# alexbuburuzan/MObI

Measured on AMD Instinct MI355X. Metric: denoising throughput (UNet element-forwards/s = steps/s x UNet batch), higher is better.
Workload: dtype bf16; 1 GPU; mobi_nusc_512 UNet denoising step, 8 objects/GPU (UNet batch 16), latent 64x64, DDIM-50 schedule, cfg_scale 1.0; objects_per_gpu=8, unet_batch=16, latent=64, sampler=ddim, parallelism=dp1 (objects sharded, no collective in the loop)

## Files before the change

mobi_amd/csrc/igemm.hip:

```cpp
#include <stdlib.h>

#include <type_traits>

#include "common.h"
#include "tuning.h"
#include "igemm_small.h"

#ifndef MOBI_FRAG2
#define MOBI_FRAG2 0
#endif
#ifndef MOBI_DMA_KS
#define MOBI_DMA_KS 1
#endif
#if defined(MOBI_IGEMM_FENCE) && MOBI_IGEMM_FENCE
#define MOBI_SCHED_FENCE() __builtin_amdgcn_sched_barrier(0)
#else
#define MOBI_SCHED_FENCE() ((void)0)
#endif

#ifndef MOBI_DBG_SKIP
#define MOBI_DBG_SKIP 0
#endif
#ifndef MOBI_PP_DMA_KS
#define MOBI_PP_DMA_KS 1
// ... 37 lines not shown
__device__ unsigned long long* g_phase = nullptr;
#define MOBI_PHASE_DECL unsigned long long ph_t[6]; unsigned ph_acc[5] = {0u, 0u, 0u, 0u, 0u}; unsigned ph_n = 0
#define MOBI_PHASE(i) ph_t[i] = __builtin_amdgcn_s_memrealtime()
#define MOBI_PHASE_ACC()                                                                  \
  do {                                                                                    \
    for (int i_ = 0; i_ < 5; ++i_) ph_acc[i_] += (unsigned)(ph_t[i_ + 1] - ph_t[i_]);     \
    ++ph_n;                                                                               \
  } while (0)
#else
#define MOBI_PHASE_DECL ((void)0)
#define MOBI_PHASE(i) ((void)0)
#define MOBI_PHASE_ACC() ((void)0)
#endif

#if MOBI_STAMP == 5
#define MOBI_SP_ENTRY const unsigned long long sp_t0 = __builtin_amdgcn_s_memtime()
#define MOBI_SP_DECL unsigned long long sp_t[7], sp_acc[6] = {0, 0, 0, 0, 0, 0}, sp_n = 0, sp_first = 0, sp_last = 0
#define MOBI_SP(i) sp_t[i] = __builtin_amdgcn_s_memtime()
#define MOBI_SP_ACC()                                                              \
  do {                                                                             \
    for (int i_ = 0; i_ < 6; ++i_) sp_acc[i_] += sp_t[i_ + 1] - sp_t[i_];          \
    if (!sp_n) sp_first = sp_t[0];                                                 \
    sp_last = sp_t[6];                                                             \
    ++sp_n;                                                                        \
  } while (0)
#define MOBI_SP_WRITE()                                                                                                   \
  do {                                                                                                                    \
    asm volatile("s_waitcnt vmcnt(0)" ::: "memory");                                                                      \
    const unsigned long long sp_end = __builtin_amdgcn_s_memtime();                                                       \
    if (g_phase && lane == 0) {                                                                                           \
      unsigned long long* d_ = g_phase + ((size_t)(blockIdx.x + gridDim.x * (blockIdx.y + gridDim.y * blockIdx.z)) * 8 + wave * 2) * 8; \
      for (int i_ = 0; i_ < 6; ++i_) d_[i_] = sp_acc[i_];                                                                 \
      d_[6] = sp_n; d_[7] = sp_end - sp_t0;                                                                               \
      d_[8] = sp_n ? sp_first - sp_t0 : 0; d_[9] = sp_n ? sp_end - sp_last : 0;                                           \
    }                                                                                                                     \
  } while (0)
#else
#define MOBI_SP_ENTRY ((void)0)
#define MOBI_SP_DECL ((void)0)
#define MOBI_SP(i) ((void)0)
#define MOBI_SP_ACC() ((void)0)
#define MOBI_SP_WRITE() ((void)0)
#endif

__device__ __attribute__((aligned(16))) unsigned int g_zero16[4] = {0u, 0u, 0u, 0u};

struct IgemmArgs {
  const void* src0; const void* src1;
  int c0, c1, C;
  int hin, win, up, hout, wout, hw_out;
  int kh, kw, stride, pad_h, pad_w;
  int img_pix_stride;
  const void* weight; long long w_group_stride;
  int n_packed, cout, ktot, nk;
  int M;
  int imgs_per_group;
  const float* bias; const float* rowvec; int rowvec_stride;
  const void* residual; long long res_img_stride;
  void* out; long long out_img_stride;
  int out_mode, epilogue;
  float scale;
  int tiles_m, tiles_n;
  int n_major;
  int src0_bytes, src1_bytes, w_bytes, fast, glds;
  int k_order;
  int wm;
  int splits, nk_per;
  float* split_ws;
  const float* ln_svec;
  float ln_eps;
  int sync_mode;
  int* sync;
  int ring_direct;
  int sm_direct;
  const void* w_tiled;
  int sm64;
  int lin_window;
  int epi_direct;
  int pp;
  int sm;
  int wide;
  int hw_shift, w_shift;
  int small;
};

#define MOBI_TILE_OF_M(L_, tile_m_, tile_n_) const int tile_n_ = (L_) % a.tiles_n, tile_m_ = (L_) / a.tiles_n
#define MOBI_TILE_OF(L_, tile_m_, tile_n_)                                                     \
  const int tdiv_##tile_m_ = __builtin_amdgcn_readfirstlane(a.n_major ? a.tiles_m : a.tiles_n); \
  const int tq_##tile_m_ = (L_) / tdiv_##tile_m_, tr_##tile_m_ = (L_) - tq_##tile_m_ * tdiv_##tile_m_; \
  const int tile_m_ = a.n_major ? tr_##tile_m_ : tq_##tile_m_;                                 \
  const int tile_n_ = a.n_major ? tq_##tile_m_ : tr_##tile_m_


__device__ __forceinline__ void vm_store16_dev(void* p, const u32x4& v);

template <int RPP, bool TR, int NT>
struct EpiGeom {
  static constexpr int WAVE_N = NT * 16;
  static constexpr int STRIDE = TR ? (RPP + 4) : (WAVE_N + 4);
  static constexpr int ROWS = TR ? WAVE_N : RPP;
  static constexpr int BYTES = ROWS * STRIDE * 4;
};

template <typename T, int NT, bool TR, int RPP, bool RES_EARLY = true, bool LEAKY = false>
__device__ __forceinline__ void igemm_epilogue(const IgemmArgs& a, float* stage, f32x4 (&acc)[NT][4], int lane,
                                               int group, int nw0, int mw0) {
  constexpr int WAVE_N = NT * 16;
  constexpr int STAGE_STRIDE = EpiGeom<RPP, TR, NT>::STRIDE;
  constexpr int MT = RPP / 16;
  constexpr int NPASS = 4 / MT;
  const int r16 = lane & 15, g4 = lane >> 4;
  const float scale = a.scale;
  T* __restrict__ outT = reinterpret_cast<T*>(a.out);
  float* __restrict__ outF = reinterpret_cast<float*>(a.out);
  const T* __restrict__ resid = reinterpret_cast<const T*>(a.residual);
  const bool plain = !TR && !a.split_ws && a.epilogue != MOBI_EPI_GEGLU;
  const bool use_bias = a.bias != nullptr && !a.split_ws;

  const int mw0c = mw0 < a.M ? mw0 : 0;
  const int img0 = __builtin_amdgcn_readfirstlane(mw0c / a.hw_out);
  const int rem0 = mw0c - img0 * a.hw_out;
  auto locate = [&](int row_in_tile, int& img, int& rem) {
    img = img0; rem = rem0 + row_in_tile;
    while (rem >= a.hw_out) { rem -= a.hw_out; ++img; }
  };

  f32x4 bias4[NT];
#pragma unroll
  for (int ni = 0; ni < NT; ++ni) {
    bias4[ni] = f32x4{0.f, 0.f, 0.f, 0.f};
    if (use_bias) {
      if (!TR) {
        const int n = nw0 + ni * 16 + g4 * 4;
        if (n < a.n_packed) bias4[ni] = *reinterpret_cast<const f32x4*>(a.bias + n);
      } else {
        const int n = nw0 + ni * 16 + r16;
        const float b = n < a.cout ? a.bias[n] : 0.f;
        bias4[ni] = f32x4{b, b, b, b};
      }
    }
  }

  constexpr int TPR_P = WAVE_N / 8;
  constexpr int NIT_P = (RPP * TPR_P + 63) / 64;
  u32x4 rres[RES_EARLY ? NPASS : 1][NIT_P];
  auto request_rows = [&](int pass, u32x4 (&dst)[NIT_P]) {
#pragma unroll
    for (int it = 0; it < NIT_P; ++it) {
      dst[it] = u32x4{0u, 0u, 0u, 0u};
      const int task = lane + 64 * it;
      const int row = task / TPR_P, cg = task - row * TPR_P;
      const int rt = pass * RPP + row;
      const int n = nw0 + cg * 8;
      if (task < RPP * TPR_P && mw0 + rt < a.M && n < a.cout) {
        int img, rem;
        locate(rt, img, rem);
        const long long gi = (long long)(group * a.imgs_per_group + img);
        dst[it] = ld16(resid + gi * a.res_img_stride + (long long)rem * a.cout + n);
      }
    }
  };
  if (RES_EARLY && plain && resid) {
#pragma unroll
    for (int pass = 0; pass < NPASS; ++pass) request_rows(pass, rres[pass]);
  }

// ... 199 lines not shown
      const int img = m / a.hw_out, rem = m - img * a.hw_out;
      if (a.bias) {
        float bb[8];
        ld8f(a.bias + n, bb);
#pragma unroll
        for (int j = 0; j < 8; ++j) o[j] += bb[j];
      }
      if (a.rowvec) {
        float rv[8];
        ld8f(a.rowvec + (long long)img * a.rowvec_stride + n, rv);
#pragma unroll
        for (int j = 0; j < 8; ++j) o[j] += rv[j];
      }
      if (resid) {
        float rf[8];
        unpack8<T>(ld16(resid + (long long)img * a.res_img_stride + (long long)rem * a.cout + n), rf);
#pragma unroll
        for (int j = 0; j < 8; ++j) o[j] += rf[j];
      }
      const long long off = (long long)img * a.out_img_stride + (long long)rem * a.cout + n;
      if (a.out_mode == MOBI_OUT_ROWS_F32) {
        *reinterpret_cast<f32x4*>(outF + off) = f32x4{o[0], o[1], o[2], o[3]};
        *reinterpret_cast<f32x4*>(outF + off + 4) = f32x4{o[4], o[5], o[6], o[7]};
      } else {
        st16(outT + off, pack8<T>(o));
      }
    }
  }
}

template <typename T, int THREADS>
__device__ __forceinline__ void splitk_arrive_and_finish(const IgemmArgs& a, int tile, int m0, int bm, int n0, int bn, int* s_flag) {
  asm volatile("s_waitcnt vmcnt(0)" ::: "memory");
  __syncthreads();
  if (threadIdx.x == 0) {
    *s_flag = a.sync_mode == 2 ? __hip_atomic_fetch_add(a.sync + tile, 1, __ATOMIC_RELAXED, __HIP_MEMORY_SCOPE_WORKGROUP)
                               : __hip_atomic_fetch_add(a.sync + tile, 1, __ATOMIC_RELAXED, __HIP_MEMORY_SCOPE_AGENT);
  }
  __syncthreads();
  if (*s_flag != a.splits - 1) return;
  if (threadIdx.x == 0) {
    if (a.sync_mode == 2) __hip_atomic_store(a.sync + tile, 0, __ATOMIC_RELAXED, __HIP_MEMORY_SCOPE_WORKGROUP);
    else __hip_atomic_store(a.sync + tile, 0, __ATOMIC_RELAXED, __HIP_MEMORY_SCOPE_AGENT);
  }
  if (a.sync_mode == 2) splitk_finish_tile<T, THREADS, false>(a, m0, bm, n0, bn);
  else splitk_finish_tile<T, THREADS, true>(a, m0, bm, n0, bn);
}

__device__ __forceinline__ void wait_vmcnt_le(int n) {
#define MOBI_VMW(k) else if (n >= k) asm volatile("s_waitcnt vmcnt(" #k ")" ::: "memory")
  if (n >= 37) asm volatile("s_waitcnt vmcnt(37)" ::: "memory");
  MOBI_VMW(32); MOBI_VMW(27); MOBI_VMW(26); MOBI_VMW(22); MOBI_VMW(18); MOBI_VMW(17); MOBI_VMW(14); MOBI_VMW(12);
  MOBI_VMW(10); MOBI_VMW(8); MOBI_VMW(7); MOBI_VMW(6); MOBI_VMW(5); MOBI_VMW(4);
  else asm volatile("s_waitcnt vmcnt(0)" ::: "memory");
#undef MOBI_VMW
}

#ifndef MOBI_PP_GEGLU_STORE16
#define MOBI_PP_GEGLU_STORE16 1
#endif
#ifndef MOBI_PP_WDUP
#define MOBI_PP_WDUP 0
#endif
#ifndef MOBI_PP_FASTWAIT
#define MOBI_PP_FASTWAIT 1
#endif
__device__ __forceinline__ void wait_vmcnt_le_fast(int n) {
  if (!MOBI_PP_FASTWAIT) { wait_vmcnt_le(n); return; }
  if (n == 7) asm volatile("s_waitcnt vmcnt(7)" ::: "memory");
  else if (n == 6) asm volatile("s_waitcnt vmcnt(6)" ::: "memory");
  else wait_vmcnt_le(n);
}

#define MOBI_SWAP4(INSN, X, Y)                                                                                       \
  asm volatile("s_nop 1\n\t" INSN " %0, %4\n\t" INSN " %1, %5\n\t" INSN " %2, %6\n\t" INSN " %3, %7\n\ts_nop 1" \
               : "+v"(X[0]), "+v"(X[1]), "+v"(X[2]), "+v"(X[3]), "+v"(Y[0]), "+v"(Y[1]), "+v"(Y[2]), "+v"(Y[3]))

template <int NT>
struct DirectEpiRegs {
  u32x4 bias[NT];
  u32x4 res[NT][2];
};

template <typename T, int NT, bool VEC = true, bool RES = true>
__device__ __forceinline__ int direct_epilogue_request(const IgemmArgs& a, DirectEpiRegs<NT>& q, int lane, int group,
                                                       int nw0, int mw0) {
  const int r16 = lane & 15, g4 = lane >> 4;
  int n_issued = 0;
  if (VEC && (a.bias || a.rowvec)) {
    const float* vec = a.bias;
    if (a.rowvec) {
      const int img = __builtin_amdgcn_readfirstlane(mw0 / a.hw_out);
      vec = a.rowvec + (long long)(group * a.imgs_per_group + img) * a.rowvec_stride;
    }
#pragma unroll
    for (int ni = 0; ni < NT; ++ni) q.bias[ni] = vm_load16(vec + nw0 + ni * 16 + g4 * 4);
    n_issued += NT;
  }
  if (RES && a.residual) {
    const T* __restrict__ resid = reinterpret_cast<const T*>(a.residual);
#pragma unroll
    for (int p = 0; p < 2; ++p) {
      const int m = mw0 + (2 * p + (g4 & 1)) * 16 + r16;
      const int img = m / a.hw_out, rem = m - img * a.hw_out;
      const T* rowp = resid + (long long)(group * a.imgs_per_group + img) * a.res_img_stride + (long long)rem * a.cout +
                      nw0 + 8 * (g4 >> 1);
#pragma unroll
      for (int ni = 0; ni < NT; ++ni) q.res[ni][p] = vm_load16(rowp + ni * 16);
    }
    n_issued += 2 * NT;
  }
  return n_issued;
}

template <typename T, int NT, bool GEGLU, bool VEC = true>
__device__ __forceinline__ int direct_epilogue(const IgemmArgs& a, f32x4 (&acc)[NT][4], DirectEpiRegs<NT>& q, int lane,
                                               int group, int nw0, int mw0) {
  const int r16 = lane & 15, g4 = lane >> 4;
  const float scale = a.scale;
  T* __restrict__ outT = reinterpret_cast<T*>(a.out);
  const bool has_vec = VEC && (a.bias || a.rowvec);
  if (has_vec) {
#pragma unroll
    for (int ni = 0; ni < NT; ++ni) asm volatile("" : "+v"(q.bias[ni]));
  }
  if (!GEGLU && a.residual) {
#pragma unroll
    for (int ni = 0; ni < NT; ++ni) { asm volatile("" : "+v"(q.res[ni][0])); asm volatile("" : "+v"(q.res[ni][1])); }
  }
  constexpr bool geglu = GEGLU;
#pragma unroll
  for (int p = 0; p < 2; ++p) {
    const int mi = geglu ? 2 * p + (g4 >> 1) : 2 * p + (g4 & 1);
    const int m = mw0 + mi * 16 + r16;
    const int img = m / a.hw_out, rem = m - img * a.hw_out;
    T* rowp = outT + (long long)(group * a.imgs_per_group + img) * a.out_img_stride + (long long)rem * a.cout;
#pragma unroll
    for (int ni = 0; ni < NT; ++ni) {
      f32x4 x = acc[ni][2 * p] * scale, y = acc[ni][2 * p + 1] * scale;
      if (has_vec) {
        const f32x4 b = __builtin_bit_cast(f32x4, q.bias[ni]);
        x += b; y += b;
      }
      float xs[4] = {x[0], x[1], x[2], x[3]}, ys[4] = {y[0], y[1], y[2], y[3]};
      if constexpr (geglu) MOBI_SWAP4("v_permlane32_swap_b32", xs, ys);
      else MOBI_SWAP4("v_permlane16_swap_b32", xs, ys);
      if constexpr (geglu) {
        float o[4];
#pragma unroll
        for (int r = 0; r < 4; ++r) o[r] = xs[r] * gelu_erf_f(ys[r]);
        vm_store8(rowp + (nw0 >> 1) + ni * 8 + 4 * (g4 & 1), pack4<T>(o));
      } else {
        float o[8] = {xs[0], xs[1], xs[2], xs[3], ys[0], ys[1], ys[2], ys[3]};
        if (a.residual) {
          float rf[8];
          unpack8<T>(q.res[ni][p], rf);
#pragma unroll
          for (int j = 0; j < 8; ++j) o[j] += rf[j];
        }
        vm_store16(rowp + nw0 + ni * 16 + 8 * (g4 >> 1), pack8<T>(o));
      }
    }
  }
  return 2 * NT;
}

template <typename T, int NT, bool GEGLU>
__device__ __forceinline__ void ring_register_epilogue(const IgemmArgs& a, f32x4 (&acc)[NT][8], int lane, int group, int nw0,
                                                       int mw0) {
  const int r16 = lane & 15, g4 = lane >> 4;
  T* __restrict__ outT = reinterpret_cast<T*>(a.out);
  const T* __restrict__ resid = reinterpret_cast<const T*>(a.residual);
  const bool has_res = !GEGLU && a.residual;
  u32x4 res[2][NT];
#pragma unroll
  for (int ni = 0; ni < NT; ++ni) res[0][ni] = res[1][ni] = u32x4{0u, 0u, 0u, 0u};
  auto out_row = [&](int k) {
    const int mi = GEGLU ? 2 * k + (g4 >> 1) : 2 * k + (g4 & 1);
    return mw0 + mi * 16 + r16;
  };
  auto request_res = [&](int k, u32x4 (&r)[NT]) {
    const int m = out_row(k);
    const int img = m / a.hw_out, rem = m - img * a.hw_out;
    const T* rowp = resid + (long long)(group * a.imgs_per_group + img) * a.res_img_stride + (long long)rem * a.cout + nw0 +
                    8 * (g4 >> 1);
#pragma unroll
    for (int ni = 0; ni < NT; ++ni) r[ni] = vm_load16(rowp + ni * 16);
// ... 1132 lines not shown
      if (g_stamps && threadIdx.x == 0) {
        unsigned long long* d = g_stamps + (size_t)(blockIdx.x + gridDim.x * (blockIdx.y + gridDim.y * blockIdx.z)) * 8;
        unsigned hw, xcc;
        asm volatile("s_getreg_b32 %0, hwreg(HW_REG_HW_ID)" : "=s"(hw));
        asm volatile("s_getreg_b32 %0, hwreg(HW_REG_XCC_ID)" : "=s"(xcc));
        d[4] = ((unsigned long long)xcc << 32) | hw;
        d[5] = (unsigned long long)(ks_end - ks_begin);
        d[6] = 1;
      }
#endif
      return;
    }
  }
  asm volatile("s_waitcnt vmcnt(0)" ::: "memory");
  __syncthreads();
  float* stage = reinterpret_cast<float*>(lds) + wave * (STAGE_BYTES / 4);
#pragma unroll
  for (int h = 0; h < MT / 4; ++h) {
    f32x4 part[NT][4];
#pragma unroll
    for (int i = 0; i < NT; ++i)
#pragma unroll
      for (int j = 0; j < 4; ++j) part[i][j] = acc[i][4 * h + j];
    igemm_epilogue<T, NT, TR, 32, MT == 4, LEAKY>(a, stage, part, lane, group, n0 + wn * WAVE_N, m0 + wm * MT * 16 + 64 * h);
  }
  if constexpr (!TR) {
    if (a.split_ws && a.sync) {
      splitk_arrive_and_finish<T, NW * 64>(a, tile_m * a.tiles_n + tile_n, m0, BM, n0, BN, &s_arrive);
    }
  }
#if MOBI_STAMP
  asm volatile("s_waitcnt vmcnt(0)" ::: "memory");
  MOBI_STAMP_AT(3);
  if (g_stamps && threadIdx.x == 0) {
    unsigned long long* d = g_stamps + (size_t)(blockIdx.x + gridDim.x * (blockIdx.y + gridDim.y * blockIdx.z)) * 8;
    unsigned hw, xcc;
    asm volatile("s_getreg_b32 %0, hwreg(HW_REG_HW_ID)" : "=s"(hw));
    asm volatile("s_getreg_b32 %0, hwreg(HW_REG_XCC_ID)" : "=s"(xcc));
    d[4] = ((unsigned long long)xcc << 32) | hw;
    d[5] = (unsigned long long)(ks_end - ks_begin);
    d[6] = 1;
  }
#endif
}

template <typename T, int NT, bool TR, bool LNF = false, bool OVL = false>
__global__ __launch_bounds__(256, 1) void igemm_ring64_kernel(const IgemmArgs a) {
  typedef typename Vec8<T>::type frag_t;
  constexpr int NW = 4, MT = 4, BM = 128, SL = 4;
  constexpr int APW = BM / 8 / NW;
  constexpr int WAVE_N = NT * 16;
  constexpr int BN = 2 * WAVE_N;
  constexpr int SLOT = (BM + BN) * 128;
  constexpr int RING = SL * SLOT;
  constexpr int STAGE_BYTES = EpiGeom<32, TR, NT>::BYTES;
  constexpr int LDS_BYTES = RING > NW * STAGE_BYTES ? RING : NW * STAGE_BYTES;
  constexpr unsigned OOB = 0x80000000u;
  constexpr int TAIL_BYTES = OVL ? 16 + (LNF ? BM * 2 * 4 : 0) : 0;
  __shared__ __attribute__((aligned(16))) unsigned char lds[LDS_BYTES + TAIL_BYTES];
  __shared__ int s_arrive_obj;
  __shared__ float s_rowstat_obj[LNF ? BM * 2 : 2];
  int* const s_arrive = OVL ? reinterpret_cast<int*>(lds + LDS_BYTES) : &s_arrive_obj;
  float* const s_rowstat = OVL ? reinterpret_cast<float*>(lds + LDS_BYTES + 16) : s_rowstat_obj;
  static_assert(!(LNF && TR), "the LayerNorm fold has no transposed-output form");
  typedef __attribute__((address_space(3))) void* lds_ptr_t;

  MOBI_SP_ENTRY;
  const int tid = threadIdx.x, lane = tid & 63, wave = tid >> 6;
  const int wave_s = __builtin_amdgcn_readfirstlane(wave);
  const int wm = wave & 1, wn = wave >> 1;
  const int group = blockIdx.z;
  const int nblk = a.tiles_m * a.tiles_n;
  const int L = xcd_remap(blockIdx.x, nblk);
  MOBI_TILE_OF(L, tile_m, tile_n);
  const int m0 = tile_m * BM, n0 = tile_n * BN;
  const T* wgt = reinterpret_cast<const T*>(a.weight) + (long long)group * a.w_group_stride;
  const __amdgpu_buffer_rsrc_t rx0 = __builtin_amdgcn_make_buffer_rsrc(const_cast<void*>(a.src0), 0, a.src0_bytes, 0x00020000);
  const __amdgpu_buffer_rsrc_t rx1 =
      __builtin_amdgcn_make_buffer_rsrc(const_cast<void*>(a.src1 ? a.src1 : a.src0), 0, a.src1 ? a.src1_bytes : 0, 0x00020000);
  const __amdgpu_buffer_rsrc_t rw = __builtin_amdgcn_make_buffer_rsrc(const_cast<T*>(wgt), 0, a.w_bytes, 0x00020000);

  const int rp = lane >> 3;
  const unsigned chunk16 = (unsigned)((lane & 7) ^ rp) * 16u;
  int x_base[APW], x_h[APW], x_w[APW];
  bool x_ok[APW];
#pragma unroll
  for (int j = 0; j < APW; ++j) {
    const int m = m0 + 8 * (APW * wave + j) + rp;
    x_ok[j] = m < a.M;
    const int mm = x_ok[j] ? m : 0;
    const int img = mm / a.hw_out, rem = mm - img * a.hw_out;
    const int ho = rem / a.wout, wo = rem - ho * a.wout;
    x_base[j] = (group * a.imgs_per_group + img) * a.img_pix_stride;
    x_h[j] = ho * a.stride - a.pad_h;
    x_w[j] = wo * a.stride - a.pad_w;
  }
  unsigned w_off[NT];
#pragma unroll
  for (int i = 0; i < NT; ++i) {
    const int n = n0 + 8 * (wave + NW * i) + rp;
    w_off[i] = n < a.n_packed ? (unsigned)n * (unsigned)a.ktot * 2u + chunk16 : OOB;
  }
  const int hlog = a.hin << a.up, wlog = a.win << a.up;
  const int ks_all = a.ktot >> 6;
  const int ks_begin = blockIdx.y * a.nk_per;
  const int ks_end = min(ks_all, ks_begin + a.nk_per);
  int u_c, u_tap, u_ky, u_kx;
  {
    const long long c_first = (long long)ks_begin * 64;
    u_tap = (int)(c_first / a.C); u_c = (int)(c_first - (long long)u_tap * a.C);
    u_ky = u_tap / a.kw; u_kx = u_tap - u_ky * a.kw;
  }
  unsigned f_row[APW];
#pragma unroll
  for (int j = 0; j < APW; ++j) f_row[j] = OOB;
  int f_tap = -1, f_src = -1, f_ks = ks_begin;

  unsigned char* p_st = lds;
  bool p_live = false;
  int p_src = 0, p_soff = 0, p_kb = 0;
  auto prep_step = [&]() __attribute__((always_inline)) {
    p_st = lds + (f_ks & (SL - 1)) * SLOT;
    p_live = f_ks < ks_end;
    const int src = u_c >= a.c0 ? 1 : 0;
    if (p_live && (u_tap != f_tap || src != f_src)) {
      f_tap = u_tap; f_src = src;
      const unsigned cs2 = (unsigned)(src ? a.c1 : a.c0) * 2u;
#pragma unroll
      for (int j = 0; j < APW; ++j) {
        const int hi = x_h[j] + u_ky, wi = x_w[j] + u_kx;
        const bool ok = x_ok[j] && (unsigned)hi < (unsigned)hlog && (unsigned)wi < (unsigned)wlog;
        f_row[j] = ok ? (unsigned)(x_base[j] + (hi >> a.up) * a.win + (wi >> a.up)) * cs2 + chunk16 : OOB;
      }
    }
    p_src = src;
    p_soff = (src ? u_c - a.c0 : u_c) * 2;
    p_kb = f_ks * 128;
    ++f_ks;
    if (p_live) {
      u_c += 64;
      if (u_c >= a.C) { u_c = 0; ++u_tap; if (++u_kx == a.kw) { u_kx = 0; ++u_ky; } }
    }
  };
  auto req_x = [&](int j) __attribute__((always_inline)) {
    const unsigned vo = p_live ? f_row[j] : OOB;
    if (p_src) __builtin_amdgcn_raw_ptr_buffer_load_lds(rx1, (lds_ptr_t)(p_st + 8 * (APW * wave_s + j) * 128), 16, vo, p_soff, 0, 0);
    else       __builtin_amdgcn_raw_ptr_buffer_load_lds(rx0, (lds_ptr_t)(p_st + 8 * (APW * wave_s + j) * 128), 16, vo, p_soff, 0, 0);
  };
  auto issue_step = [&]() {
    prep_step();
#pragma unroll
    for (int j = 0; j < APW; ++j) req_x(j);
#pragma unroll
    for (int i = 0; i < NT; ++i) {
      const unsigned vo = p_live ? w_off[i] : OOB;
      __builtin_amdgcn_raw_ptr_buffer_load_lds(rw, (lds_ptr_t)(p_st + BM * 128 + 8 * (wave_s + NW * i) * 128), 16, vo, p_kb, 0, 0);
    }
  };
  auto wait_step = [&]() {
    if (NT == 5) asm volatile("s_waitcnt vmcnt(18)" ::: "memory"); else asm volatile("s_waitcnt vmcnt(16)" ::: "memory");
  };

  f32x4 acc[NT][MT];
#pragma unroll
  for (int i = 0; i < NT; ++i)
#pragma unroll
    for (int j = 0; j < MT; ++j) acc[i][j] = f32x4{0.f, 0.f, 0.f, 0.f};
  constexpr int SPW = MT / (NW / 2);
  constexpr bool lnf = LNF;
  float ls_sum[SPW], ls_sq[SPW];
#pragma unroll
  for (int i = 0; i < SPW; ++i) ls_sum[i] = ls_sq[i] = 0.f;

  const int r16 = lane & 15, g4 = lane >> 4;
  const unsigned char* xrd = lds + (wm * 64 + r16) * 128;
  const unsigned char* wrd = lds + BM * 128 + (wn * WAVE_N + r16) * 128;

  MOBI_SP_DECL;
  if constexpr (OVL) {
    auto req = [&](int g) __attribute__((always_inline)) {
      if (g < APW) { req_x(g); return; }
      const int i = g - APW;
      const unsigned vo = p_live ? w_off[i] : OOB;
      __builtin_amdgcn_raw_ptr_buffer_load_lds(rw, (lds_ptr_t)(p_st + BM * 128 + 8 * (wave_s + NW * i) * 128), 16, vo, p_kb, 0, 0);
    };
    issue_step(); issue_step(); issue_step();
    auto k_loop = [&](auto wnc) __attribute__((always_inline)) {
      constexpr int WNC = decltype(wnc)::value;
#pragma clang loop unroll(disable)
      for (int s = ks_begin; s < ks_end; ++s) {
        MOBI_SP(0);
        wait_step();
        MOBI_SP(1);
        __builtin_amdgcn_sched_barrier(0);
        __builtin_amdgcn_s_barrier();
        __builtin_amdgcn_sched_barrier(0);
        MOBI_SP(2);
        const int so = (s & (SL - 1)) * SLOT;
        frag_t xf[2][MT], wf[2][NT];
#pragma unroll
        for (int ks = 0; ks < 2; ++ks) {
          const int sw = ((ks * 4 + g4) ^ (r16 & 7)) << 4;
#pragma unroll
          for (int mi = 0; mi < MT; ++mi) xf[ks][mi] = __builtin_bit_cast(frag_t, ld16(xrd + so + mi * 16 * 128 + sw));
#pragma unroll
          for (int ni = 0; ni < NT; ++ni) wf[ks][ni] = __builtin_bit_cast(frag_t, ld16(wrd + so + ni * 16 * 128 + sw));
        }
        prep_step();
        __builtin_amdgcn_sched_barrier(0);
        MOBI_SP(3);
#if MOBI_STAMP == 5
        sp_t[4] = sp_t[5] = sp_t[3];
#endif
#pragma unroll
        for (int ks = 0; ks < 2; ++ks)
#pragma unroll
          for (int ni = 0; ni < NT; ++ni) {
#pragma unroll
            for (int mi = 0; mi < MT; ++mi) {
              acc[ni][mi] = TR ? mfma16(xf[ks][mi], wf[ks][ni], acc[ni][mi]) : mfma16(wf[ks][ni], xf[ks][mi], acc[ni][mi]);
              if constexpr (lnf) if (ni == 0 && mi < SPW) rowstat_acc(xf[ks][SPW * WNC + mi], ls_sum[mi], ls_sq[mi]);
            }
            __builtin_amdgcn_sched_barrier(0);
            if (ks * NT + ni < APW + NT) req(ks * NT + ni);
            __builtin_amdgcn_sched_barrier(0);
          }
        MOBI_SP(6);
        MOBI_SP_ACC();
      }
    };
    if constexpr (lnf) {
      if ((wave_s >> 1) == 0) k_loop(std::integral_constant<int, 0>{}); else k_loop(std::integral_constant<int, 1>{});
    } else {
      k_loop(std::integral_constant<int, 0>{});
    }
  } else {
  issue_step(); issue_step(); issue_step();
  auto k_loop = [&](auto wnc) {
  constexpr int WNC = decltype(wnc)::value;
#pragma clang loop unroll(disable)
  for (int s = ks_begin; s < ks_end; ++s) {
    MOBI_SP(0);
    wait_step();
    MOBI_SP(1);
    __builtin_amdgcn_sched_barrier(0);
    __builtin_amdgcn_s_barrier();
    __builtin_amdgcn_sched_barrier(0);
    MOBI_SP(2);
    const int so = (s & (SL - 1)) * SLOT;
    frag_t xf[2][MT], wf[2][NT];
#pragma unroll
    for (int ks = 0; ks < 2; ++ks) {
      const int sw = ((ks * 4 + g4) ^ (r16 & 7)) << 4;
#pragma unroll
      for (int mi = 0; mi < MT; ++mi) xf[ks][mi] = __builtin_bit_cast(frag_t, ld16(xrd + so + mi * 16 * 128 + sw));
#pragma unroll
      for (int ni = 0; ni < NT; ++ni) wf[ks][ni] = __builtin_bit_cast(frag_t, ld16(wrd + so + ni * 16 * 128 + sw));
    }
    __builtin_amdgcn_sched_barrier(0);
    MOBI_SP(3);
    issue_step();
    __builtin_amdgcn_sched_barrier(0);
    MOBI_SP(4);
    asm volatile("s_waitcnt lgkmcnt(0)" ::: "memory");
    MOBI_SP(5);
    __builtin_amdgcn_s_setprio(1);
#pragma unroll
    for (int ks = 0; ks < 2; ++ks)
#pragma unroll
      for (int ni = 0; ni < NT; ++ni)
#pragma unroll
        for (int mi = 0; mi < MT; ++mi) {
          acc[ni][mi] = TR ? mfma16(xf[ks][mi], wf[ks][ni], acc[ni][mi]) : mfma16(wf[ks][ni], xf[ks][mi], acc[ni][mi]);
          if constexpr (lnf) if (ni == 0 && mi < SPW) rowstat_acc(xf[ks][SPW * WNC + mi], ls_sum[mi], ls_sq[mi]);
        }
    if constexpr (lnf) {
#pragma unroll
      for (int i = 0; i < 16 * SPW; ++i) {
        __builtin_amdgcn_sched_group_barrier(0x008, 1, 0);
        __builtin_amdgcn_sched_group_barrier(0x002, 1, 0);
      }
#pragma unroll
      for (int i = 0; i < SPW; ++i) asm volatile("" : "+v"(ls_sum[i]), "+v"(ls_sq[i]));
    }
    __builtin_amdgcn_s_setprio(0);
    MOBI_SP(6);
    MOBI_SP_ACC();
  }
  };
  if constexpr (lnf) {
    if ((wave_s >> 1) == 0) k_loop(std::integral_constant<int, 0>{}); else k_loop(std::integral_constant<int, 1>{});
  } else {
    k_loop(std::integral_constant<int, 0>{});
  }
  }
  if constexpr (lnf) ln_fold_acc<NT, MT, SPW>(a, acc, ls_sum, ls_sq, s_rowstat, lane, wm, wave_s >> 1, n0 + wn * WAVE_N, false);
  if constexpr (!TR) {
    if (a.sm_direct) {
      asm volatile("s_waitcnt vmcnt(0)" ::: "memory");
      const int nw0 = n0 + wn * WAVE_N, mw0 = m0 + wm * 64;
      if (a.split_ws) {
        float* wsp = a.split_ws + (long long)blockIdx.y * a.M * a.n_packed;
#pragma unroll
        for (int mi = 0; mi < 4; ++mi) {
          float* rowp = wsp + (long long)(mw0 + mi * 16 + r16) * a.n_packed + nw0 + g4 * 4;
#pragma unroll
          for (int ni = 0; ni < NT; ++ni) slab_store16(a.sync_mode == 1, rowp + ni * 16, __builtin_bit_cast(u32x4, acc[ni][mi]));
        }
        if (a.sync) {
          splitk_arrive_and_finish<T, NW * 64>(a, tile_m * a.tiles_n + tile_n, m0, BM, n0, BN, s_arrive);
        }
      } else {
        DirectEpiRegs<NT> q;
#pragma unroll
        for (int ni = 0; ni < NT; ++ni) { q.bias[ni] = u32x4{0u, 0u, 0u, 0u}; q.res[ni][0] = q.res[ni][1] = u32x4{0u, 0u, 0u, 0u}; }
        direct_epilogue_request<T, NT>(a, q, lane, group, nw0, mw0);
        asm volatile("s_waitcnt vmcnt(0)" ::: "memory");
        if (a.epilogue == MOBI_EPI_GEGLU) direct_epilogue<T, NT, true>(a, acc, q, lane, group, nw0, mw0);
        else direct_epilogue<T, NT, false>(a, acc, q, lane, group, nw0, mw0);
      }
      MOBI_SP_WRITE();
      return;
    }
  }
  asm volatile("s_waitcnt vmcnt(0)" ::: "memory");
  __syncthreads();
  float* stage = reinterpret_cast<float*>(lds) + wave * (STAGE_BYTES / 4);
  igemm_epilogue<T, NT, TR, 32, true>(a, stage, acc, lane, group, n0 + wn * WAVE_N, m0 + wm * 64);
  if constexpr (!TR) {
    if (a.split_ws && a.sync) {
      splitk_arrive_and_finish<T, NW * 64>(a, tile_m * a.tiles_n + tile_n, m0, BM, n0, BN, s_arrive);
    }
  }
  MOBI_SP_WRITE();
}

template <typename T>
__global__ __launch_bounds__(256) void igemm_splitk_reduce_kernel(const IgemmArgs a) {
  const int vpr = a.cout >> 3;
  const long long total = (long long)a.M * vpr;
  T* __restrict__ outT = reinterpret_cast<T*>(a.out);
  float* __restrict__ outF = reinterpret_cast<float*>(a.out);
  const T* __restrict__ resid = reinterpret_cast<const T*>(a.residual);
  for (long long i = (long long)blockIdx.x * 256 + threadIdx.x; i < total; i += (long long)gridDim.x * 256) {
    const int m = (int)(i / vpr);
    const int n = (int)(i - (long long)m * vpr) * 8;
    float o[8];
#pragma unroll
    for (int j = 0; j < 8; ++j) o[j] = 0.f;
    const long long slab = (long long)a.M * a.n_packed;
    const float* p0 = a.split_ws + (long long)m * a.n_packed + n;
    int s = 0;
    for (; s + 4 <= a.splits; s += 4) {
      f32x4 v[4][2];
#pragma unroll
      for (int u = 0; u < 4; ++u) {
        const float* p = p0 + (s + u) * slab;
        v[u][0] = *reinterpret_cast<const f32x4*>(p);
        v[u][1] = *reinterpret_cast<const f32x4*>(p + 4);
      }
#pragma unroll
      for (int u = 0; u < 4; ++u)
#pragma unroll
        for (int j = 0; j < 4; ++j) { o[j] += v[u][0][j]; o[4 + j] += v[u][1][j]; }
    }
    for (; s < a.splits; ++s) {
      const float* p = p0 + s * slab;
      const f32x4 v0 = *reinterpret_cast<const f32x4*>(p), v1 = *reinterpret_cast<const f32x4*>(p + 4);
#pragma unroll
      for (int j = 0; j < 4; ++j) { o[j] += v0[j]; o[4 + j] += v1[j]; }
    }
    const int img = m / a.hw_out, rem = m - img * a.hw_out;
    if (a.bias) {
      float bb[8];
      ld8f(a.bias + n, bb);
#pragma unroll
      for (int j = 0; j < 8; ++j) o[j] += bb[j];
    }
    if (a.rowvec) {
      float rv[8];
      ld8f(a.rowvec + (long long)img * a.rowvec_stride + n, rv);
#pragma unroll
      for (int j = 0; j < 8; ++j) o[j] += rv[j];
    }
    if (resid) {
      float rf[8];
      unpack8<T>(ld16(resid + (long long)img * a.res_img_stride + (long long)rem * a.cout + n), rf);
#pragma unroll
      for (int j = 0; j < 8; ++j) o[j] += rf[j];
    }
    const long long off = (long long)img * a.out_img_stride + (long long)rem * a.cout + n;
    if (a.out_mode == MOBI_OUT_ROWS_F32) {
      *reinterpret_cast<f32x4*>(outF + off) = f32x4{o[0], o[1], o[2], o[3]};
      *reinterpret_cast<f32x4*>(outF + off + 4) = f32x4{o[4], o[5], o[6], o[7]};
    } else {
      st16(outT + off, pack8<T>(o));
    }
  }
}

// ... 268 lines not shown
    a.split_ws = reinterpret_cast<float*>(p->ws);
  }
  if (p->defer_finish != 0 && p->defer_finish != 1) return MOBI_ERR_ARG;
  if (p->defer_finish && (!a.split_ws || p->sync || p->out_mode != MOBI_OUT_ROWS)) return MOBI_ERR_UNSUPPORTED;
  a.lin_window = 0;
  a.epi_direct = a.wm == 4 && a.fast && a.glds && p->out_mode == MOBI_OUT_ROWS && !a.split_ws &&
                 (!p->rowvec || (!p->bias && a.hw_out % 64 == 0)) && a.M % 256 == 0 && p->n_packed % bn == 0 &&
                 a.nk_per >= 3;
  if (tuning().epi_direct == 0) a.epi_direct = 0;
  auto log2_exact = [](int v) { int s = 0; while ((1 << s) < v) ++s; return (1 << s) == v ? s : -1; };
  a.hw_shift = log2_exact(a.hw_out); a.w_shift = log2_exact(a.wout);
  a.pp = a.epi_direct && a.splits == 1 && p->scale == 1.0f && a.hw_shift >= 6 && a.w_shift >= 0 &&
         a.hout < 32768 && a.wout < 32768;
  if (a.split_ws && a.wm == 4 && a.fast && a.glds && p->out_mode != MOBI_OUT_TRANSPOSED && a.M % 256 == 0 &&
      p->n_packed % bn == 0 && a.nk_per >= 3 && p->scale == 1.0f && a.hw_shift >= 6 && a.w_shift >= 0 &&
      a.hout < 32768 && a.wout < 32768)
    a.pp = 1;
  if (tuning().pp == 0) a.pp = 0;
  a.wide = 0;
  if ((a.wm == 4 || tuning().wide > 0) && ring_ok && tuning().wide != 0) {
    const int bnw = (p->n_packed % 160) == 0 ? 320 : 256;
    const long long tn = (p->n_packed + bnw - 1) / bnw;
    auto fills = [&](long long blocks) {
      const long long rounds = (blocks + 255) / 256;
      return blocks >= 190 && blocks * 5 >= rounds * 256 * 4 - 64 * (rounds == 1);
    };
    const long long t256 = ((a.M + 255) / 256) * tn * a.splits, t128 = ((a.M + 127) / 128) * tn * a.splits;
    int pick = tuning().wide > 0 ? tuning().wide : (fills(t256) ? 2 : (fills(t128) && tuning().wide128 == 1 ? 1 : 0));
    if (tuning().wide <= 0 && pick == 2 && p->n_packed * 2 <= bnw && a.pp) pick = 0;
    if (!pick && a.wm == 4 && !a.pp && (a.C >= 64 || p->out_mode != MOBI_OUT_ROWS || p->n_packed < 256)) pick = 2;
    if (lnf) pick = a.wm == 4 ? 2 : 0;
    if (pick) {
      a.wide = pick;
      a.wm = pick == 2 ? 4 : 2;
      a.tiles_m = (a.M + 64 * a.wm - 1) / (64 * a.wm);
      a.tiles_n = (int)tn;
      a.sm = 0;
    }
  }
  {
    const long long wbytes = (long long)p->n_packed * a.ktot * 2;
    const long long abytes = (long long)p->batch * p->hin * p->win * a.C * 2;
    a.n_major = p->groups == 1 && a.tiles_n >= 2 && p->kh * p->kw == 1 && wbytes > abytes && tuning().n_major != 0;
    if (tuning().n_major == 1 && p->groups == 1) a.n_major = 1;
    if (!a.wide && a.wm == 4 && a.fast && a.glds && a.pp) a.n_major = 0;
  }
  a.sm64 = a.sm && a.C % 64 == 0 && (p->c1 == 0 || p->c0 % 64 == 0) && a.nk_per >= 1 &&
           (long long)a.tiles_m * a.tiles_n * a.splits * p->groups <= (long long)compute_units() && tuning().sm64 != 0;
  if (tuning().sm64 == 1 && a.sm && a.C % 64 == 0 && (p->c1 == 0 || p->c0 % 64 == 0)) a.sm64 = 1;
  a.w_tiled = (p->weight_tiled && !a.sm64 && (a.sm || a.wide) &&
               (p->groups == 1 || p->w_group_stride == (long long)p->n_packed * a.ktot) && p->n_packed % 16 == 0 &&
               a.ktot % 32 == 0 && !(reinterpret_cast<uintptr_t>(p->weight_tiled) & 15) && tuning().w_tiled != 0)
                  ? p->weight_tiled : nullptr;
  a.sm_direct = (a.sm || a.wide == 1) && (p->out_mode == MOBI_OUT_ROWS || a.split_ws) && p->out_mode != MOBI_OUT_TRANSPOSED &&
                a.M % 128 == 0 && p->n_packed % (a.wide == 1 ? 2 * bn : bn) == 0 &&
                (a.split_ws || !p->rowvec || (!p->bias && a.hw_out % 64 == 0)) && tuning().sm_direct != 0;
  {
    const int bnw = (p->n_packed % 160) == 0 ? 320 : 256;
    a.ring_direct = a.wide == 2 && p->out_mode == MOBI_OUT_ROWS && !a.split_ws && p->groups == 1 &&
                    (!p->rowvec || (!p->bias && a.hw_out % 128 == 0)) && a.M % 256 == 0 && p->n_packed % bnw == 0 &&
                    p->scale == 1.0f && !p->residual && tuning().ring_direct != 0;
    if (tuning().ring_direct == 1 && p->residual && a.wide == 2 && p->out_mode == MOBI_OUT_ROWS && !a.split_ws && p->groups == 1 &&
        (!p->rowvec || (!p->bias && a.hw_out % 128 == 0)) && a.M % 256 == 0 && p->n_packed % bnw == 0 && p->scale == 1.0f)
      a.ring_direct = 1;
  }
  if (leaky) {
    if (!ring_ok) return MOBI_ERR_UNSUPPORTED;
    a.pp = 0; a.epi_direct = 0; a.sm_direct = 0; a.ring_direct = 0; a.sm64 = 0; a.n_major = 0;
    if (a.wm == 4 && p->n_packed >= 256) {
      const int bnw = (p->n_packed % 160) == 0 ? 320 : 256;
      a.wide = 2; a.sm = 0;
      a.tiles_m = (a.M + 255) / 256;
      a.tiles_n = (p->n_packed + bnw - 1) / bnw;
    } else {
      a.wide = 0; a.wm = 2; a.sm = 1;
      a.tiles_m = (a.M + 127) / 128;
      a.tiles_n = (p->n_packed + bn - 1) / bn;
    }
    a.w_tiled = (p->weight_tiled && (p->groups == 1 || p->w_group_stride == (long long)p->n_packed * a.ktot) &&
                 p->n_packed % 16 == 0 && a.ktot % 32 == 0 && !(reinterpret_cast<uintptr_t>(p->weight_tiled) & 15) &&
                 tuning().w_tiled != 0) ? p->weight_tiled : nullptr;
    if ((long long)a.tiles_m * a.tiles_n > 0x7fffffffLL) return MOBI_ERR_UNSUPPORTED;
  }
  a.small = lnf || leaky ? 0 : small_tile(p);
  if (lnf && !(a.wide || a.sm)) return MOBI_ERR_UNSUPPORTED;
  a.sync = nullptr; a.sync_mode = 0;
  if (a.split_ws && p->sync && !a.small && tuning().fused_split != 0 && a.splits <= 4 &&
      (long long)a.splits * a.M * a.n_packed * 4 < 0x7fffffffLL) {
    if (reinterpret_cast<uintptr_t>(p->sync) & 3) return MOBI_ERR_ALIGN;
    const long long tiles = (long long)a.tiles_m * a.tiles_n;
    const bool pp_launch = !a.wide && a.wm == 4 && a.fast && a.glds && a.pp;
    const bool ring_launch = a.wide || a.sm;
    const int mode = tuning().fused_split == 1 ? 1 : 2;
    if ((ring_launch || (pp_launch && tiles <= (long long)compute_units())) && (mode == 1 || tiles % 8 == 0)) {
      a.sync = reinterpret_cast<int*>(p->sync);
      a.sync_mode = mode;
    }
  }
  return MOBI_OK;
}

static int launch_small(const mobi_igemm_params* p, const mobi::IgemmArgs& a, hipStream_t st) {
  mobi::SmallGemmArgs s;
  s.src0 = a.src0; s.src1 = a.src1; s.c0 = a.c0; s.c1 = a.c1;
  s.taps = a.kh * a.kw; s.hin = a.hin; s.win = a.win;
  s.hw = a.hw_out; s.img_pix_stride = a.img_pix_stride;
  s.weight = a.weight;
  s.M = a.M; s.N = a.n_packed; s.K = a.ktot;
  s.bias = a.bias; s.rowvec = a.rowvec; s.rowvec_stride = a.rowvec_stride;
  s.residual = a.residual; s.res_img_stride = a.res_img_stride;
  s.out = a.out; s.out_img_stride = a.out_img_stride; s.out_f32 = a.out_mode == MOBI_OUT_ROWS_F32;
  s.scale = a.scale;
  s.tiles_m = (a.M + a.small - 1) / a.small; s.tiles_n = a.n_packed / a.small;
  const long long wbytes = (long long)a.n_packed * a.ktot * 2, abytes = (long long)a.M * a.ktot * 2;
  s.n_major = wbytes > abytes;
  return mobi::launch_small_gemm(s, p->dtype, st);
}

extern "C" int mobi_igemm(const mobi_igemm_params* p, void* stream) {
  using namespace mobi;
  IgemmArgs a;
  const int rc = igemm_prepare(p, a);
  if (rc != MOBI_OK) return rc;
  hipStream_t st = reinterpret_cast<hipStream_t>(stream);
  if (a.small) return launch_small(p, a, st);
  return p->dtype == MOBI_F16 ? launch_igemm<f16_t>(p, a, p->groups, st) : launch_igemm<bf16_t>(p, a, p->groups, st);
}

extern "C" int32_t mobi_igemm_slab_count(const mobi_igemm_params* p) {
  mobi::IgemmArgs a;
  const int rc = igemm_prepare(p, a);
  if (rc != MOBI_OK) return rc;
  return a.small ? 1 : a.splits;
}

extern "C" int mobi_igemm_finish(const mobi_igemm_params* p, void* stream) {
  using namespace mobi;
  IgemmArgs a;
  const int rc = igemm_prepare(p, a);
  if (rc != MOBI_OK) return rc;
  if (!a.split_ws || a.small || a.sync) return MOBI_ERR_ARG;
  hipStream_t st = reinterpret_cast<hipStream_t>(stream);
  return p->dtype == MOBI_F16 ? launch_splitk_reduce<f16_t>(a, st) : launch_splitk_reduce<bf16_t>(a, st);
}

extern "C" int mobi_igemm_kernel_variant(const mobi_igemm_params* p) {
  mobi::IgemmArgs a;
  const int rc = igemm_prepare(p, a);
  if (rc != MOBI_OK) return rc;
  if (a.small) return MOBI_IGEMM_SMALL;
  if (a.wide) return a.wide == 2 ? MOBI_IGEMM_RING_256 : MOBI_IGEMM_RING_128W;
  if (a.wm == 4 && a.fast && a.glds) return a.pp ? MOBI_IGEMM_PINGPONG : MOBI_IGEMM_DIRECT_LDS;
  if (a.wm == 4) return MOBI_IGEMM_STAGED_256;
  return a.sm ? MOBI_IGEMM_RING_128 : MOBI_IGEMM_STAGED_128;
}
```

mobi_amd/csrc/tuning.h:

```cpp
#pragma once
namespace mobi {
struct Tuning {
  int persist_blocks;
  int pp_split;
  int wm;
  int fast;
  int glds;
  int epi_direct;
  int pp;
  int sm;
  int wide;
  int wide128;
  int ring_direct;
  int sm_direct;
  int w_tiled;
  int n_major;
  int sm64;
  int sm64_ovl;
  int split_target;
  int fused_split;
  int split_longk;
  int split_round4;
  int attn_bwd_exact_d;
  int small;
  int small_mflop;
  int small_conv_m;
  int tka_mfma;
  int attn_nw;
  int tka_rows;
  int attn_nw8_blocks;
  int attn_h16;
  int attn_xcd;
  int cout_mfma;
  int skinny_mfma;
  int gn_coop;
  int gn_fused;
  int gn_split_pw4;
  int attn_v3;
};
const Tuning& tuning();
}
```

mobi_amd/csrc/tuning.hip:

```cpp
#include <atomic>
#include <cstdlib>
#include <mutex>

#include "common.h"
#include "tuning.h"

namespace mobi {
namespace {
Tuning g_tuning;
std::once_flag g_once;

int env_int(const char* name) {
  const char* e = getenv(name);
  return (e && e[0]) ? atoi(e) : -1;
}
void read_env() {
  g_tuning.persist_blocks = env_int("MOBI_IGEMM_PERSIST_BLOCKS");
  g_tuning.pp_split = env_int("MOBI_IGEMM_PP_SPLIT");
  g_tuning.wm = env_int("MOBI_IGEMM_WM");
  g_tuning.fast = env_int("MOBI_IGEMM_FAST");
  g_tuning.glds = env_int("MOBI_IGEMM_GLDS");
  g_tuning.epi_direct = env_int("MOBI_IGEMM_EPI_DIRECT");
  g_tuning.pp = env_int("MOBI_IGEMM_PP");
  g_tuning.sm = env_int("MOBI_IGEMM_SM");
  g_tuning.wide = env_int("MOBI_IGEMM_WIDE");
  g_tuning.wide128 = env_int("MOBI_IGEMM_WIDE128");
  g_tuning.ring_direct = env_int("MOBI_IGEMM_RING_DIRECT");
  g_tuning.sm_direct = env_int("MOBI_IGEMM_SM_DIRECT");
  g_tuning.w_tiled = env_int("MOBI_IGEMM_WTILED");
  g_tuning.sm64 = env_int("MOBI_IGEMM_SM64");
  g_tuning.sm64_ovl = env_int("MOBI_IGEMM_SM64_OVL");
  g_tuning.n_major = env_int("MOBI_IGEMM_N_MAJOR");
  g_tuning.split_target = env_int("MOBI_IGEMM_SPLIT_TARGET");
  g_tuning.split_longk = env_int("MOBI_IGEMM_SPLIT_LONGK");
  g_tuning.split_round4 = env_int("MOBI_IGEMM_SPLIT_ROUND4");
  g_tuning.attn_bwd_exact_d = env_int("MOBI_ATTN_BWD_EXACT_D");
  g_tuning.fused_split = env_int("MOBI_IGEMM_FUSED_SPLIT");
  g_tuning.small = env_int("MOBI_IGEMM_SMALL");
  g_tuning.small_mflop = env_int("MOBI_IGEMM_SMALL_MFLOP");
  g_tuning.small_conv_m = env_int("MOBI_IGEMM_SMALL_CONV_M");
  g_tuning.tka_mfma = env_int("MOBI_TKA_MFMA");
  g_tuning.attn_nw = env_int("MOBI_ATTN_NW");
  g_tuning.attn_v3 = env_int("MOBI_ATTN_V3");
  g_tuning.gn_fused = env_int("MOBI_GN_FUSED");
  g_tuning.gn_coop = env_int("MOBI_GN_COOP");
  g_tuning.gn_split_pw4 = env_int("MOBI_GN_SPLIT_PW4");
  g_tuning.skinny_mfma = env_int("MOBI_SKINNY_MFMA");
  g_tuning.cout_mfma = env_int("MOBI_COUT_MFMA");
  g_tuning.attn_xcd = env_int("MOBI_ATTN_XCD");
  g_tuning.attn_h16 = env_int("MOBI_ATTN_H16");
  g_tuning.attn_nw8_blocks = env_int("MOBI_ATTN_NW8_BLOCKS");
  g_tuning.tka_rows = env_int("MOBI_TKA_ROWS");
}
}

const Tuning& tuning() {
  std::call_once(g_once, read_env);
  return g_tuning;
}
}

extern "C" int mobi_tuning_reload(void) {
  std::call_once(mobi::g_once, [] {});
  mobi::read_env();
  return MOBI_OK;
}

extern "C" int mobi_build_info(void) { return 0; }
```

Measured before the change: 842.9 UNet element-forwards/s.

## Issue first weight tile and epilogue operand loads at implicit-GEMM kernel entry

At kernel start, the implicit-GEMM kernel now issues the first k-step's weight loads into LDS before the per-row address setup. For direct-epilogue, non-split tiles it also requests the bias, row-vector and residual loads at that point. The aim is to hide the start-of-kernel latency and the final epilogue load wait behind address computation and the k-loop. For 1x1 stride-1 convolutions it also replaces per-row divides with linear or shift-based row addressing. The risk is that the epilogue registers stay live across the whole k-loop, which raises register pressure and may reduce occupancy. The path is on by default because an unset environment variable reads as -1, which counts as enabled.

```diff
diff --git a/mobi_amd/csrc/igemm.hip b/mobi_amd/csrc/igemm.hip
--- a/mobi_amd/csrc/igemm.hip
+++ b/mobi_amd/csrc/igemm.hip
@@ -143,6 +143,8 @@
   int wide;
   int hw_shift, w_shift;
   int small;
+  int entry_req;
+  int lin_rows;
 };
 
 #define MOBI_TILE_OF_M(L_, tile_m_, tile_n_) const int tile_n_ = (L_) % a.tiles_n, tile_m_ = (L_) / a.tiles_n
@@ -508,15 +510,16 @@
   u32x4 res[NT][2];
 };
 
-template <typename T, int NT, bool VEC = true, bool RES = true>
+template <typename T, int NT, bool VEC = true, bool RES = true, bool SHIFT = false>
 __device__ __forceinline__ int direct_epilogue_request(const IgemmArgs& a, DirectEpiRegs<NT>& q, int lane, int group,
                                                        int nw0, int mw0) {
   const int r16 = lane & 15, g4 = lane >> 4;
   int n_issued = 0;
+  const bool pow2 = SHIFT && a.hw_shift >= 0;
   if (VEC && (a.bias || a.rowvec)) {
     const float* vec = a.bias;
     if (a.rowvec) {
-      const int img = __builtin_amdgcn_readfirstlane(mw0 / a.hw_out);
+      const int img = __builtin_amdgcn_readfirstlane(pow2 ? mw0 >> a.hw_shift : mw0 / a.hw_out);
       vec = a.rowvec + (long long)(group * a.imgs_per_group + img) * a.rowvec_stride;
     }
 #pragma unroll
@@ -528,7 +531,7 @@
 #pragma unroll
     for (int p = 0; p < 2; ++p) {
       const int m = mw0 + (2 * p + (g4 & 1)) * 16 + r16;
-      const int img = m / a.hw_out, rem = m - img * a.hw_out;
+      const int img = pow2 ? m >> a.hw_shift : m / a.hw_out, rem = m - img * a.hw_out;
       const T* rowp = resid + (long long)(group * a.imgs_per_group + img) * a.res_img_stride + (long long)rem * a.cout +
                       nw0 + 8 * (g4 >> 1);
 #pragma unroll
@@ -1827,6 +1830,33 @@
 
   const int rp = lane >> 3;
   const unsigned chunk16 = (unsigned)((lane & 7) ^ rp) * 16u;
+  const bool entry = a.entry_req != 0;
+  const int ks_all = a.ktot >> 6;
+  const int ks_begin = blockIdx.y * a.nk_per;
+  const int ks_end = min(ks_all, ks_begin + a.nk_per);
+  unsigned w_off[NT];
+#pragma unroll
+  for (int i = 0; i < NT; ++i) {
+    const int n = n0 + 8 * (wave + NW * i) + rp;
+    w_off[i] = n < a.n_packed ? (unsigned)n * (unsigned)a.ktot * 2u + chunk16 : OOB;
+  }
+  DirectEpiRegs<NT> q;
+#pragma unroll
+  for (int ni = 0; ni < NT; ++ni) { q.bias[ni] = u32x4{0u, 0u, 0u, 0u}; q.res[ni][0] = q.res[ni][1] = u32x4{0u, 0u, 0u, 0u}; }
+  bool epi_at_entry = false;
+  if constexpr (!TR) {
+    epi_at_entry = entry && a.sm_direct && !a.split_ws;
+    if (epi_at_entry) direct_epilogue_request<T, NT, true, true, true>(a, q, lane, group, n0 + wn * WAVE_N, m0 + wm * 64);
+  }
+  if (entry) {
+    unsigned char* st = lds + (ks_begin & (SL - 1)) * SLOT;
+    const bool live = ks_begin < ks_end;
+#pragma unroll
+    for (int i = 0; i < NT; ++i) {
+      const unsigned vo = live ? w_off[i] : OOB;
+      __builtin_amdgcn_raw_ptr_buffer_load_lds(rw, (lds_ptr_t)(st + BM * 128 + 8 * (wave_s + NW * i) * 128), 16, vo, ks_begin * 128, 0, 0);
+    }
+  }
   int x_base[APW], x_h[APW], x_w[APW];
   bool x_ok[APW];
 #pragma unroll
@@ -1834,24 +1864,21 @@
     const int m = m0 + 8 * (APW * wave + j) + rp;
     x_ok[j] = m < a.M;
     const int mm = x_ok[j] ? m : 0;
-    const int img = mm / a.hw_out, rem = mm - img * a.hw_out;
-    const int ho = rem / a.wout, wo = rem - ho * a.wout;
-    x_base[j] = (group * a.imgs_per_group + img) * a.img_pix_stride;
-    x_h[j] = ho * a.stride - a.pad_h;
-    x_w[j] = wo * a.stride - a.pad_w;
-  }
-  unsigned w_off[NT];
-#pragma unroll
-  for (int i = 0; i < NT; ++i) {
-    const int n = n0 + 8 * (wave + NW * i) + rp;
-    w_off[i] = n < a.n_packed ? (unsigned)n * (unsigned)a.ktot * 2u + chunk16 : OOB;
+    if (a.lin_rows) {
+      x_base[j] = a.lin_rows == 1 ? group * a.M + mm
+                                  : (group * a.imgs_per_group + (mm >> a.hw_shift)) * a.img_pix_stride + (mm & (a.hw_out - 1));
+      x_h[j] = x_w[j] = 0;
+    } else {
+      const int img = mm / a.hw_out, rem = mm - img * a.hw_out;
+      const int ho = rem / a.wout, wo = rem - ho * a.wout;
+      x_base[j] = (group * a.imgs_per_group + img) * a.img_pix_stride;
+      x_h[j] = ho * a.stride - a.pad_h;
+      x_w[j] = wo * a.stride - a.pad_w;
+    }
   }
   const int hlog = a.hin << a.up, wlog = a.win << a.up;
-  const int ks_all = a.ktot >> 6;
-  const int ks_begin = blockIdx.y * a.nk_per;
-  const int ks_end = min(ks_all, ks_begin + a.nk_per);
-  int u_c, u_tap, u_ky, u_kx;
-  {
+  int u_c = 0, u_tap = 0, u_ky = 0, u_kx = 0;
+  if (!entry || ks_begin) {
     const long long c_first = (long long)ks_begin * 64;
     u_tap = (int)(c_first / a.C); u_c = (int)(c_first - (long long)u_tap * a.C);
     u_ky = u_tap / a.kw; u_kx = u_tap - u_ky * a.kw;
@@ -1902,6 +1929,16 @@
       __builtin_amdgcn_raw_ptr_buffer_load_lds(rw, (lds_ptr_t)(p_st + BM * 128 + 8 * (wave_s + NW * i) * 128), 16, vo, p_kb, 0, 0);
     }
   };
+  auto issue_head = [&]() __attribute__((always_inline)) {
+    if (entry) {
+      prep_step();
+#pragma unroll
+      for (int j = 0; j < APW; ++j) req_x(j);
+    } else {
+      issue_step();
+    }
+    issue_step(); issue_step();
+  };
   auto wait_step = [&]() {
     if (NT == 5) asm volatile("s_waitcnt vmcnt(18)" ::: "memory"); else asm volatile("s_waitcnt vmcnt(16)" ::: "memory");
   };
@@ -1929,7 +1966,7 @@
       const unsigned vo = p_live ? w_off[i] : OOB;
       __builtin_amdgcn_raw_ptr_buffer_load_lds(rw, (lds_ptr_t)(p_st + BM * 128 + 8 * (wave_s + NW * i) * 128), 16, vo, p_kb, 0, 0);
     };
-    issue_step(); issue_step(); issue_step();
+    issue_head();
     auto k_loop = [&](auto wnc) __attribute__((always_inline)) {
       constexpr int WNC = decltype(wnc)::value;
 #pragma clang loop unroll(disable)
@@ -1980,7 +2017,7 @@
       k_loop(std::integral_constant<int, 0>{});
     }
   } else {
-  issue_step(); issue_step(); issue_step();
+  issue_head();
   auto k_loop = [&](auto wnc) {
   constexpr int WNC = decltype(wnc)::value;
 #pragma clang loop unroll(disable)
@@ -2056,11 +2093,10 @@
           splitk_arrive_and_finish<T, NW * 64>(a, tile_m * a.tiles_n + tile_n, m0, BM, n0, BN, s_arrive);
         }
       } else {
-        DirectEpiRegs<NT> q;
-#pragma unroll
-        for (int ni = 0; ni < NT; ++ni) { q.bias[ni] = u32x4{0u, 0u, 0u, 0u}; q.res[ni][0] = q.res[ni][1] = u32x4{0u, 0u, 0u, 0u}; }
-        direct_epilogue_request<T, NT>(a, q, lane, group, nw0, mw0);
-        asm volatile("s_waitcnt vmcnt(0)" ::: "memory");
+        if (!epi_at_entry) {
+          direct_epilogue_request<T, NT>(a, q, lane, group, nw0, mw0);
+          asm volatile("s_waitcnt vmcnt(0)" ::: "memory");
+        }
         if (a.epilogue == MOBI_EPI_GEGLU) direct_epilogue<T, NT, true>(a, acc, q, lane, group, nw0, mw0);
         else direct_epilogue<T, NT, false>(a, acc, q, lane, group, nw0, mw0);
       }
@@ -2495,6 +2531,11 @@
                  tuning().w_tiled != 0) ? p->weight_tiled : nullptr;
     if ((long long)a.tiles_m * a.tiles_n > 0x7fffffffLL) return MOBI_ERR_UNSUPPORTED;
   }
+  a.entry_req = tuning().entry_req != 0;
+  a.lin_rows = 0;
+  if (a.entry_req && p->kh == 1 && p->kw == 1 && p->stride == 1 && !p->pad_h && !p->pad_w && !p->upsample && p->hout == p->hin &&
+      p->wout == p->win)
+    a.lin_rows = ips == hw_in ? 1 : (a.hw_shift >= 0 ? 2 : 0);
   a.small = lnf || leaky ? 0 : small_tile(p);
   if (lnf && !(a.wide || a.sm)) return MOBI_ERR_UNSUPPORTED;
   a.sync = nullptr; a.sync_mode = 0;
diff --git a/mobi_amd/csrc/tuning.h b/mobi_amd/csrc/tuning.h
--- a/mobi_amd/csrc/tuning.h
+++ b/mobi_amd/csrc/tuning.h
@@ -17,6 +17,7 @@
   int n_major;
   int sm64;
   int sm64_ovl;
+  int entry_req;
   int split_target;
   int fused_split;
   int split_longk;
diff --git a/mobi_amd/csrc/tuning.hip b/mobi_amd/csrc/tuning.hip
--- a/mobi_amd/csrc/tuning.hip
+++ b/mobi_amd/csrc/tuning.hip
@@ -30,6 +30,7 @@
   g_tuning.w_tiled = env_int("MOBI_IGEMM_WTILED");
   g_tuning.sm64 = env_int("MOBI_IGEMM_SM64");
   g_tuning.sm64_ovl = env_int("MOBI_IGEMM_SM64_OVL");
+  g_tuning.entry_req = env_int("MOBI_IGEMM_ENTRY_REQ");
   g_tuning.n_major = env_int("MOBI_IGEMM_N_MAJOR");
   g_tuning.split_target = env_int("MOBI_IGEMM_SPLIT_TARGET");
   g_tuning.split_longk = env_int("MOBI_IGEMM_SPLIT_LONGK");
```

After: 844.0 UNet element-forwards/s, median of 5. About the same (+0.1%).
